# akb825/Cuttlefish

Measured on AMD Instinct MI355X. Metric: Mpixels/s encode, BC7 4096x4096 RGBA8, higher is better.
Workload: dtype u8; 1 GPU; BC7 UNORM Texture::Quality::Normal, one 4096x4096 RGBA8 synthetic photo tile per GPU, resident in HBM; format=BC7, quality=2, blocks_per_launch=1048576, parallelism=surface-per-gpu x1

## Files before the change

cuttlefish_amd/csrc/bc7_encode.hip:

```cpp
#include "cf_device.h"
#include "bc7_packed.h"
#include "bc7_rcp.h"
#include "bc7_roles.h"
#include "bc7_cand.h"

namespace {

#define CF_FRESH_LANE(x) asm volatile("v_mbcnt_lo_u32_b32 %0, -1, 0\n\tv_mbcnt_hi_u32_b32 %0, -1, %0" : "=v"(x))

__device__ __forceinline__ int cf_bperm(int v, uint32_t src)
{
	return __builtin_amdgcn_ds_bpermute((int)(src << 2), v);
}

__device__ const cf_bc7_role_table k_bc7_roles = cf_bc7_make_roles();

__device__ const cf_bc7_cand_table k_bc7_cands = cf_bc7_make_cands();
__device__ const cf_bc7_mask_table k_bc7_masks = cf_bc7_make_masks();

__device__ const cf_bc7_weight_table k_bc7_weights = cf_bc7_make_weights();

__device__ const uint16_t k_part2[64] = CF_BC7_PART2_INIT;

__device__ const uint8_t k_anchor2[64] = {
// ... 216 lines not shown
}

__device__ __forceinline__ uint32_t dot2_u16(uint32_t a, uint32_t b, uint32_t acc)
{
	return __builtin_amdgcn_udot2(__builtin_bit_cast(cf_us2, a), __builtin_bit_cast(cf_us2, b), acc, false);
}

__device__ __forceinline__ void ycc_pairs(uint32_t r, uint32_t g, uint32_t b, uint32_t a, uint32_t& prg, uint32_t& pba)
{
	const uint32_t y = (109u*r + 366u*g + 37u*b + 256u) >> 9;
	prg = y | ((r + 255u - y) << 16);
	pba = (b + 255u - y) | (a << 16);
}

__device__ __forceinline__ uint32_t ycc_pp_sum(const Tex& tx, uint32_t mask, const uint32_t (&yw)[2])
{
	uint32_t pp = 0;
#pragma unroll 1
	for (uint32_t r = 0; r < 4u; ++r) {
		const uint4 ya = *reinterpret_cast<const uint4*>(tx.yc() + 8u*r);
		const uint4 yb = *reinterpret_cast<const uint4*>(tx.yc() + 8u*r + 4u);
		const uint32_t pr[8] = {ya.x, ya.y, ya.z, ya.w, yb.x, yb.y, yb.z, yb.w};
#pragma unroll
		for (int j = 0; j < 4; ++j) {
			const uint32_t t = dot2_u16(pk_mul_u16(pr[2*j], yw[0]), pr[2*j], dot2_u16(pk_mul_u16(pr[2*j + 1], yw[1]), pr[2*j + 1], 0u));
			pp += ((mask >> (4u*r + (uint32_t)j)) & 1u) ? t : 0u;
		}
	}
	return pp;
}

#ifndef CF_BC7_ABLATE
#define CF_BC7_ABLATE 0
#endif
#ifndef CF_BC7_CANDW
#define CF_BC7_CANDW 1
#endif
#ifndef CF_BC7_FITTRIMS
#define CF_BC7_FITTRIMS 3
#endif

#ifndef CF_BC7_DIAG
#define CF_BC7_DIAG 0
#endif
#if CF_BC7_DIAG
enum { CF_DIAG_STARTS, CF_DIAG_STARTS_CACHED, CF_DIAG_STARTS_NARROW, CF_DIAG_PERTURB, CF_DIAG_PERTURB_NARROW,
	CF_DIAG_STARTS_NOPB, CF_DIAG_PERTURB_NOPB, CF_DIAG_PERTURB_PPHIT, CF_DIAG_N };
__device__ unsigned long long cf_bc7_diag[CF_DIAG_N];
#define CF_DIAG_COUNT(i, cond) do { uint32_t l_; CF_FRESH_LANE(l_); if (l_ == 0u && (cond)) atomicAdd(&cf_bc7_diag[i], 1ull); } while (0)
#else
#define CF_DIAG_COUNT(i, cond) do { } while (0)
#endif

struct LaneFit {
	uint32_t q0, q1, pb, err;
	uint32_t w[4];
};

template <bool UNITW, int NK = 8>
__device__ __forceinline__ void assign_lsq_lane(const Tex& tx, uint32_t mask, bool m6,
	uint32_t khalf, uint32_t ib, const uint32_t (&yw)[2], uint32_t pp_sum, bool want_lsq, uint32_t fe0, uint32_t fe1,
	LaneFit& f, float (&nx0)[4], float (&nx1)[4], float (&hq)[3], bool& ok, uint32_t s01 = 0u, uint32_t s23 = 0u)
{
	constexpr bool MINKEY = (CF_BC7_KEYTRIMS & 1) != 0;
	const uint32_t nk = m6 ? 8u : (1u << ib), kbase = m6 ? 8u*khalf : 0u;
	const uint32_t e00 = ub(fe0, 0), e01 = ub(fe0, 1), e02 = ub(fe0, 2), e03 = ub(fe0, 3);
	const uint32_t e10 = ub(fe1, 0), e11 = ub(fe1, 1), e12 = ub(fe1, 2), e13 = ub(fe1, 3);
	uint32_t pal[8], palh[8];
	int base[8];
	uint32_t w03 = 0, w47 = 0;
	if (CF_BC7_FITTRIMS & 2) {
		const uint32_t* wr = k_bc7_weights.w[weight_row(m6, khalf, ib)];
		w03 = wr[0];
		w47 = NK == 8 ? wr[1] : 0u;
	}
	const PalLine line = pal_line(fe0, fe1);
#pragma unroll
	for (int k = 0; k < NK; ++k) {
		const bool valid = ((CF_BC7_FITTRIMS & 2) && k < 4) || (uint32_t)k < nk;
		const uint32_t w = (CF_BC7_FITTRIMS & 2) ? weight_at(w03, w47, (uint32_t)k)
			: bc7_weight(ib, valid ? kbase + (uint32_t)k : 0u);
		const uint32_t iw = 64u - w;
		if (UNITW) {
			pal[k] = (CF_BC7_FITTRIMS & 1) ? pal_at(line, w) : pal_word(fe0, fe1, w);
			palh[k] = 0;
			const int B = (int)((__builtin_amdgcn_udot4(pal[k], pal[k], 0u, false) << 7) | w);
			base[k] = MINKEY ? (valid ? B : CF_BC7_NO_ENTRY) : (valid ? -B : -CF_BC7_NO_ENTRY);
		} else {
			const uint32_t c0 = (__umul24(iw, e00) + __umul24(w, e10) + 32u) >> 6;
			const uint32_t c1 = (__umul24(iw, e01) + __umul24(w, e11) + 32u) >> 6;
			const uint32_t c2 = (__umul24(iw, e02) + __umul24(w, e12) + 32u) >> 6;
			const uint32_t c3 = (__umul24(iw, e03) + __umul24(w, e13) + 32u) >> 6;
			uint32_t qrg, qba;
			ycc_pairs(c0, c1, c2, c3, qrg, qba);
			pal[k] = pk_mul_u16(qrg, yw[0]);
			palh[k] = pk_mul_u16(qba, yw[1]);
			const uint32_t qq = dot2_u16(pal[k], qrg, dot2_u16(palh[k], qba, 0u));
			const int B = (int)((qq << 7) | w);
			base[k] = MINKEY ? (valid ? B : CF_BC7_NO_ENTRY) : (valid ? -B : -CF_BC7_NO_ENTRY);
		}
		asm volatile("" : "+v"(base[k]));
	}
	int m256 = -256;
	if (MINKEY) asm volatile("" : "+s"(m256));
	uint32_t err = pp_sum;
	uint32_t wp0 = 0, wp1 = 0, wp2 = 0, wp3 = 0;
#pragma unroll 1
	for (uint32_t r2 = 0; r2 < 4u; r2 += 2u) {
		uint32_t wpair[2];
#pragma unroll
		for (uint32_t h = 0; h < 2u; ++h) {
			const uint32_t r = r2 + h;
			uint32_t raw[4], rawh[4];
			if (UNITW) {
				const uint4 rw = *reinterpret_cast<const uint4*>(tx.tp() + 4u*r);
				raw[0] = rw.x; raw[1] = rw.y; raw[2] = rw.z; raw[3] = rw.w;
				rawh[0] = rawh[1] = rawh[2] = rawh[3] = 0u;
			} else {
				const uint4 ya = *reinterpret_cast<const uint4*>(tx.yc() + 8u*r);
				const uint4 yb = *reinterpret_cast<const uint4*>(tx.yc() + 8u*r + 4u);
				raw[0] = ya.x; raw[1] = ya.z; raw[2] = yb.x; raw[3] = yb.z;
				rawh[0] = ya.y; rawh[1] = ya.w; rawh[2] = yb.y; rawh[3] = yb.w;
			}
			const uint32_t mrow = (mask >> (4u*r)) & 15u;
			uint32_t wrow = 0;
#pragma unroll
			for (int j = 0; j < 4; ++j) {
				uint32_t rawj = raw[j];
				asm volatile("" : "+v"(rawj), "+v"(wrow));
				const uint32_t p = UNITW ? texel<true>(tx, rawj) : 0u;
				uint32_t key;
				{
					int bestk = MINKEY ? 0x7FFFFFFF : -0x7FFFFFFF;
					const uint32_t prg = rawj, pba = rawh[j];
#pragma unroll
					for (int k = 0; k < NK; ++k) {
						int dt;
						if (UNITW)
							dt = (int)__builtin_amdgcn_udot4(p, pal[k], 0u, false);
						else
							dt = (int)dot2_u16(pba, palh[k], dot2_u16(prg, pal[k], 0u));
						if (MINKEY) {
							const int v = key_min_form(dt, m256, base[k]);
							bestk = v < bestk ? v : bestk;
						} else {
							const int v = key_max_form(dt, base[k]);
							bestk = v > bestk ? v : bestk;
						}
					}
					if (NK == 8) {
						const int other = (int)cf_xor1((uint32_t)bestk);
						bestk = (m6 && (MINKEY ? other < bestk : other > bestk)) ? other : bestk;
					}
					key = (uint32_t)(MINKEY ? bestk : -bestk);
				}
				key = ((mrow >> j) & 1u) ? key : 0u;
				err += (uint32_t)((int)key >> 7);
				wrow |= (key & 127u) << (8*j);
			}
			wpair[h] = wrow;
		}
		wp0 = wp2; wp1 = wp3; wp2 = wpair[0]; wp3 = wpair[1];
	}
	f.err = err;
	f.w[0] = wp0; f.w[1] = wp1; f.w[2] = wp2; f.w[3] = wp3;
	uint32_t S = 0, A = 0, B = 0, C = 0, U[4] = {0, 0, 0, 0}, V[4] = {0, 0, 0, 0};
	if (want_lsq) {
#pragma unroll 1
		for (uint32_t r = 0; r < 4u; ++r) {
			const uint32_t wrow = wp0;
			wp0 = wp1; wp1 = wp2; wp2 = wp3; wp3 = wrow;
			uint32_t P[4];
			uint32_t bo = tx.boff;
			asm volatile("" : "+v"(bo));
			planes<true>(tx, *reinterpret_cast<const uint4*>(tx.plan_ + bo + 4u*r), P);
			S = __builtin_amdgcn_udot4(wrow, 0x01010101u, S, false);
			C = __builtin_amdgcn_udot4(wrow, wrow, C, false);
#pragma unroll
			for (int c = 0; c < 4; ++c)
				V[c] = __builtin_amdgcn_udot4(wrow, P[c], V[c], false);
		}
		A = 4096u*(uint32_t)__builtin_popcount(mask) - 128u*S + C;
		B = 64u*S - C;
		U[0] = 64u*(s01 & 0xFFFFu) - V[0]; U[1] = 64u*(s01 >> 16) - V[1];
		U[2] = 64u*(s23 & 0xFFFFu) - V[2]; U[3] = 64u*(s23 >> 16) - V[3];
	}
	const int det = (int)__umul24((uint32_t)__builtin_popcount(mask), C) - (int)__umul24(S, S);
	ok = det > 0;
	const float inv = rcp_ranged(64.0f*(float)(det > 0 ? det : 1));
	const float fA = (float)A, fB = (float)B, fC = (float)C;
#pragma unroll
	for (int c = 0; c < 4; ++c) {
		if ((tx.chmask >> c) & 1u) {
			const float fU = (float)U[c], fV = (float)V[c];
			const float t0 = fB*fV;
			const float n0 = fmaf(fC, fU, -t0);
			const float t1 = fB*fU;
			const float n1 = fmaf(fA, fV, -t1);
			nx0[c] = n0*inv;
			nx1[c] = n1*inv;
		} else {
			nx0[c] = 0.0f;
			nx1[c] = 0.0f;
		}
	}
	hq[0] = fA; hq[1] = fB; hq[2] = fC;
}

__device__ __forceinline__ void refit_window(const float (&xu0)[4], const float (&xu1)[4], const float (&hq)[3],
	uint32_t cb, uint32_t ab, uint32_t pbk, SubFit& f)
{
	const uint32_t S = pbk ? 1u : 0u;
	const uint32_t P0 = f.pb & 1u, P1 = (f.pb >> 1) & 1u;
// ... 20 lines not shown
			dl1[d] = fb(dw1[d], c) - xu1[c];
		}
		dl0[0] = (lo0 & bm) ? dl0[0] : 1.0e18f;
		dl0[2] = (hi0 & bm) ? dl0[2] : 1.0e18f;
		dl1[0] = (lo1 & bm) ? dl1[0] : 1.0e18f;
		dl1[2] = (hi1 & bm) ? dl1[2] : 1.0e18f;
		float best = 3.0e38f;
		uint32_t bi = 0x11u << (8*c);
#pragma unroll
		for (int i = 0; i < 3; ++i) {
			const float d0 = dl0[i];
			float a0 = fA*d0;
			a0 = a0*d0;
			const float cr = fB2*d0;
#pragma unroll
			for (int j = 0; j < 3; ++j) {
				const float d1 = dl1[j];
				float v = fC*d1;
				v = fmaf(v, d1, a0);
				v = fmaf(cr, d1, v);
				const bool take = v < best;
				best = take ? v : best;
				bi = take ? (uint32_t)(i | (j << 4)) << (8*c) : bi;
			}
		}
		pick |= bi;
	}
	const uint32_t nq0 = f.q0 + (pick & 0x03030303u) - 0x01010101u;
	const uint32_t nq1 = f.q1 + ((pick >> 4) & 0x03030303u) - 0x01010101u;
	const uint32_t ne0 = dequant_word(code_word(nq0, S, P0), tc, ta);
	const uint32_t ne1 = dequant_word(code_word(nq1, S, P1), tc, ta);
	f.q0 = nq0; f.q1 = nq1; f.e0 = ne0; f.e1 = ne1;
}

#define CF_BC7_GEO_WORDS 13
#define CF_BC7_GEO_NONE 0xFFFFFFFFu
__device__ __forceinline__ uint32_t geo_tag(uint32_t id, uint32_t fi) { return id*4u + (id == 0u ? 0u : fi); }

__device__ __forceinline__ uint32_t geo_src(uint32_t id, uint32_t fi, uint32_t wl, bool lay32)
{
	uint32_t s = wl + fi;
	if (id == 0u) s = wl;
	else if (id < 13u) s = fi ? wl + (lay32 ? (id < 5u ? 4u : 1u) : 12u) : wl;
	else if (lay32 && id >= 192u && id < 320u && fi == 2u)
		s = (wl & 32u) + (((wl & 31u) - 11u) >> 1);
	return s & 63u;
}

struct FitStats {
	uint32_t W[CF_MOM_WORDS];
	uint32_t lohi;
};

template <bool UNITW, uint32_t ITERS, int NK = 8, bool GIVEN = false>
__device__ __forceinline__ void fit_lane(const Tex& tx, uint32_t mask, bool m6, uint32_t khalf,
	uint32_t cb, uint32_t ab, uint32_t pbk, uint32_t ib, const uint32_t (&wt)[4],
	const uint32_t (&yw)[2], bool scalar, float frac, uint32_t* gbase, uint32_t gmode, uint32_t gsrc, const FitStats& gs, LaneFit& best)
{
	float axis[4], mean[4];
	float tmin, tmax;
	uint32_t lo, hi, pp_sum, s01, s23;
	if (gmode == 2u) {
		const uint32_t* gc = gbase + gsrc;
#pragma unroll
		for (int c = 0; c < 4; ++c) {
			axis[c] = __uint_as_float(gc[c*CF_WG_THREADS]);
			mean[c] = __uint_as_float(gc[(4 + c)*CF_WG_THREADS]);
		}
		tmin = __uint_as_float(gc[8*CF_WG_THREADS]);
		tmax = __uint_as_float(gc[9*CF_WG_THREADS]);
		const uint32_t lh = gc[10*CF_WG_THREADS];
		lo = lh & 255u; hi = lh >> 8;
		pp_sum = gc[11*CF_WG_THREADS];
		const float fn = (float)__builtin_popcount(mask);
		s01 = (uint32_t)(mean[0]*fn + 0.5f) | ((uint32_t)(mean[1]*fn + 0.5f) << 16);
		s23 = (uint32_t)(mean[2]*fn + 0.5f) | ((uint32_t)(mean[3]*fn + 0.5f) << 16);
	} else {
		const uint32_t n = (uint32_t)__builtin_popcount(mask);
		uint32_t s[4] = {0, 0, 0, 0};
		uint32_t q00 = 0, q01 = 0, q02 = 0, q03 = 0, q11 = 0, q12 = 0, q13 = 0, q22 = 0, q23 = 0,
			q33 = 0;
		lo = 255u; hi = 0u;
		if (GIVEN && gmode == 3u) {
			uint32_t q[10];
			mom_unpack(gs.W, s, q);
			q00 = q[0]; q01 = q[1]; q02 = q[2]; q03 = q[3]; q11 = q[4]; q12 = q[5]; q13 = q[6]; q22 = q[7]; q23 = q[8]; q33 = q[9];
			lo = gs.lohi & 255u; hi = gs.lohi >> 8;
		} else
#pragma unroll 1
		for (uint32_t r = 0; r < 4u; ++r) {
			uint32_t P[4];
			const uint4 pr = *reinterpret_cast<const uint4*>(tx.pl() + 4u*r);
			planes<true>(tx, pr, P);
			const uint32_t a4 = tx.rot == 0u ? pr.w : (tx.rot == 1u ? pr.x : (tx.rot == 2u ? pr.y : pr.z));
#pragma unroll
			for (int j = 0; j < 4; ++j) {
				const uint32_t a = (a4 >> (8*j)) & 255u;
				lo = a < lo ? a : lo;
				hi = a > hi ? a : hi;
			}
			const uint32_t m4 = bytemask4((mask >> (4u*r)) & 15u);
			const uint32_t M0 = P[0] & m4, M1 = P[1] & m4, M2 = P[2] & m4, M3 = P[3] & m4;
			s[0] = __builtin_amdgcn_udot4(M0, 0x01010101u, s[0], false);
			s[1] = __builtin_amdgcn_udot4(M1, 0x01010101u, s[1], false);
			s[2] = __builtin_amdgcn_udot4(M2, 0x01010101u, s[2], false);
			s[3] = __builtin_amdgcn_udot4(M3, 0x01010101u, s[3], false);
			q00 = __builtin_amdgcn_udot4(M0, P[0], q00, false);
			q01 = __builtin_amdgcn_udot4(M0, P[1], q01, false);
			q02 = __builtin_amdgcn_udot4(M0, P[2], q02, false);
			q03 = __builtin_amdgcn_udot4(M0, P[3], q03, false);
// ... 12 lines not shown

		float bestd = C00;
		float v0 = C00, v1 = C01, v2 = C02, v3 = C03;
		if (C11 > bestd) { bestd = C11; v0 = C01; v1 = C11; v2 = C12; v3 = C13; }
		if (C22 > bestd) { bestd = C22; v0 = C02; v1 = C12; v2 = C22; v3 = C23; }
		if (C33 > bestd) { bestd = C33; v0 = C03; v1 = C13; v2 = C23; v3 = C33; }
#pragma unroll
		for (int it = 0; it < 3; ++it) {
			float r0 = C00*v0; r0 = fmaf(C01, v1, r0); r0 = fmaf(C02, v2, r0); r0 = fmaf(C03, v3, r0);
			float r1 = C01*v0; r1 = fmaf(C11, v1, r1); r1 = fmaf(C12, v2, r1); r1 = fmaf(C13, v3, r1);
			float r2 = C02*v0; r2 = fmaf(C12, v1, r2); r2 = fmaf(C22, v2, r2); r2 = fmaf(C23, v3, r2);
			float r3 = C03*v0; r3 = fmaf(C13, v1, r3); r3 = fmaf(C23, v2, r3); r3 = fmaf(C33, v3, r3);
			v0 = r0; v1 = r1; v2 = r2; v3 = r3;
		}
		const float mx = fmaxf(fmaxf(fabsf(v0), fabsf(v1)), fmaxf(fabsf(v2), fabsf(v3)));
#pragma unroll
		for (int c = 0; c < 4; ++c) axis[c] = 0.0f;
		if (mx > 0.0f) {
			const float im = rcp_tested(mx);
			v0 = v0*im; v1 = v1*im; v2 = v2*im; v3 = v3*im;
			float l2 = v0*v0;
			l2 = fmaf(v1, v1, l2);
			l2 = fmaf(v2, v2, l2);
			l2 = fmaf(v3, v3, l2);
			const float is = rcp_ranged(sqrtf(l2));
			axis[0] = v0*is; axis[1] = v1*is; axis[2] = v2*is; axis[3] = v3*is;
		}

		const float in = inv_n(n);
#pragma unroll
		for (int c = 0; c < 4; ++c)
			mean[c] = (float)s[c]*in;
		tmin = 3.0e38f; tmax = -3.0e38f;
#pragma unroll 1
		for (uint32_t r = 0; r < 4u; ++r) {
			const uint4 rw = *reinterpret_cast<const uint4*>(tx.tp() + 4u*r);
			const uint32_t raw[4] = {rw.x, rw.y, rw.z, rw.w};
			const uint32_t mrow = (mask >> (4u*r)) & 15u;
#pragma unroll
			for (int j = 0; j < 4; ++j) {
				const uint32_t p = texel<true>(tx, raw[j]);
				const bool m = (mrow >> j) & 1u;
				float t = axis[0]*(fb(p, 0) - mean[0]);
				t = fmaf(axis[1], fb(p, 1) - mean[1], t);
				t = fmaf(axis[2], fb(p, 2) - mean[2], t);
				t = fmaf(axis[3], fb(p, 3) - mean[3], t);
				tmin = m ? fminf(tmin, t) : tmin;
				tmax = m ? fmaxf(tmax, t) : tmax;
			}
		}
		pp_sum = UNITW ? q00 + q11 + q22 + q33 : ycc_pp_sum(tx, mask, yw);
		s01 = s[0] | (s[1] << 16);
		s23 = s[2] | (s[3] << 16);
		if (GIVEN ? gmode != 0u : gmode == 1u) {
			uint32_t lane;
			CF_FRESH_LANE(lane);
			uint32_t* gc = gbase + lane;
#pragma unroll
			for (int c = 0; c < 4; ++c) {
				gc[c*CF_WG_THREADS] = __float_as_uint(axis[c]);
				gc[(4 + c)*CF_WG_THREADS] = __float_as_uint(mean[c]);
			}
			gc[8*CF_WG_THREADS] = __float_as_uint(tmin);
			gc[9*CF_WG_THREADS] = __float_as_uint(tmax);
			gc[10*CF_WG_THREADS] = lo | (hi << 8);
			gc[11*CF_WG_THREADS] = pp_sum;
		}
	}
	{
		const float d = (tmax - tmin)*frac;
		tmin = tmin + d;
		tmax = tmax - d;
	}
	float x0[4], x1[4];
#pragma unroll
	for (int c = 0; c < 4; ++c) {
		x0[c] = clamp255(fmaf(axis[c], tmin, mean[c]));
		x1[c] = clamp255(fmaf(axis[c], tmax, mean[c]));
	}
	if (scalar) {
		const float flo = (float)lo, fhi = (float)hi;
		const float d = (fhi - flo)*frac;
		x0[0] = 0.0f; x0[1] = 0.0f; x0[2] = 0.0f; x0[3] = clamp255(flo + d);
		x1[0] = 0.0f; x1[1] = 0.0f; x1[2] = 0.0f; x1[3] = clamp255(fhi - d);
	}
	uint32_t geo = cb | (ab << 4) | (pbk << 8) | (ib << 12);
	asm volatile("" : "+v"(geo));
#define G_CB (geo & 15u)
#define G_AB ((geo >> 4) & 15u)
#define G_PBK ((geo >> 8) & 15u)
#define G_IB (geo >> 12)
	SubFit q;
	quantize<UNITW>(x0, x1, G_CB, G_AB, G_PBK, wt, q);
	best.q0 = q.q0; best.q1 = q.q1; best.pb = q.pb;
	bool live;
	float hq[3];
	assign_lsq_lane<UNITW, NK>(tx, mask, m6, khalf, G_IB, yw, pp_sum, ITERS > 0u, q.e0, q.e1, best, x0, x1, hq, live, s01, s23);
#pragma unroll 1
	for (uint32_t r = 0; r < ITERS; ++r) {
		LaneFit cur;
		bool ok;
		asm volatile("" : "+v"(geo));
		{
			float c0[4], c1[4];
#pragma unroll
			for (int c = 0; c < 4; ++c) {
				c0[c] = clamp255(x0[c]);
				c1[c] = clamp255(x1[c]);
			}
			quantize<UNITW>(c0, c1, G_CB, G_AB, G_PBK, wt, q);
		}
		if (!(CF_BC7_ABLATE & 8)) refit_window(x0, x1, hq, G_CB, G_AB, G_PBK, q);
		cur.q0 = q.q0; cur.q1 = q.q1; cur.pb = q.pb;
		assign_lsq_lane<UNITW, NK>(tx, mask, m6, khalf, G_IB, yw, pp_sum, r + 1u < ITERS, q.e0, q.e1, cur, x0, x1, hq, ok, s01, s23);
		const bool better = live && cur.err < best.err;
		if (better)
			best = cur;
		live = better && ok;
	}
#undef G_CB
#undef G_AB
#undef G_PBK
#undef G_IB
}

__device__ __forceinline__ uint32_t w2i(uint32_t w, uint32_t ib)
{
	return (w*((1u << ib) - 1u) + 32u) >> 6;
}

__device__ __forceinline__ uint4 pack_block_group(const uint32_t* wcol, uint32_t id, uint32_t lane,
	bool pair)
{
	const uint32_t h = lane >> 5, hl = pair ? (lane & 31u) : lane, hbase = pair ? (lane & 32u) : 0u;
	if (CF_BC7_ABLATE & 64) {
		uint4 r;
		r.x = id; r.y = wcol[0]; r.z = wcol[CF_WG_THREADS]; r.w = h;
		return r;
	}
	uint32_t mode, part = 0, rot = 0, isel = 0;
	if (id == 0u) mode = 6;
	else if (id < 5u) { mode = 5; rot = id - 1u; }
	else if (id < 13u) { mode = 4; rot = (id - 5u) & 3u; isel = (id - 5u) >> 2; }
	else if (id < 128u) { mode = 1; part = id - 64u; }
	else if (id < 192u) { mode = 3; part = id - 128u; }
	else if (id < 256u) { mode = 0; part = id - 192u; }
	else if (id < 320u) { mode = 2; part = id - 256u; }
	else { mode = 7; part = id - 320u; }
	const uint32_t ns  = (0x21112323u >> (4u*mode)) & 15u;
	const uint32_t pbn = (0x60006664u >> (4u*mode)) & 15u;
	const uint32_t cb  = (0x57757564u >> (4u*mode)) & 15u;
	const uint32_t ab  = (0x57860000u >> (4u*mode)) & 15u;
	const uint32_t pk  = (0x11001021u >> (4u*mode)) & 15u;
	const uint32_t ib  = (0x24222233u >> (4u*mode)) & 15u;
	const uint32_t ib2 = (0x00230000u >> (4u*mode)) & 15u;
	uint32_t ibc = ib, iba = ib2;
	const bool swapsets = mode == 4u && isel != 0u;
	if (swapsets) { ibc = 3u; iba = 2u; }
	const uint32_t p2 = k_part2[part], p3 = k_part3[part];
	uint32_t a1 = 0, a2 = 0;
	if (ns == 2u) a1 = k_anchor2[part];
	else if (ns == 3u) { a1 = k_anchor3a[part]; a2 = k_anchor3b[part]; }

	const uint32_t t = hl & 15u;
	const uint32_t sb = ns == 1u ? 0u : (ns == 2u ? ((p2 >> t) & 1u) : ((p3 >> (2u*t)) & 3u));
	const uint32_t wv = (wcol[(7u + (t >> 2))*CF_WG_THREADS] >> (8u*(t & 3u))) & 255u;
	const uint32_t ws = (wcol[(11u + (t >> 2))*CF_WG_THREADS] >> (8u*(t & 3u))) & 255u;
// ... 576 lines not shown
					case 0: cb = 4; ab = 0; pbk = 1; ib = 3; break;
					case 2: cb = 5; ab = 0; pbk = 0; ib = 2; break;
					default: cb = 5; ab = 5; pbk = 1; ib = 2; break;
				}
				const uint32_t sp2 = k_part2[mypart], sp3 = k_part3[mypart];
				if (st == 0u)
					mask = sub ? sp2 : (~sp2 & 0xFFFFu);
				else
					mask = part3_mask(sp3, sub);
				active = true;
			}
			if (CF_BC7_ABLATE & 1) active = active && (m6 || plane);
			if (CF_BC7_ABLATE & 2) active = active && !plane;
#if CF_BC7_DIAG
			const bool nopb = __ballot(active && pbk != 0u) == 0ull;
			CF_DIAG_COUNT(CF_DIAG_STARTS_NOPB, sst && nopb);
#endif
			uint32_t wl[4] = {wt[0], wt[1], wt[2], wt[3]};
			if (!UNITW && rot) {
				const uint32_t t3 = wl[3];
				if (rot == 1u) { wl[3] = wl[0]; wl[0] = t3; }
				else if (rot == 2u) { wl[3] = wl[1]; wl[1] = t3; }
				else { wl[3] = wl[2]; wl[2] = t3; }
			}
			const uint32_t chm = (sst || words) ? chm_s : (m6 ? 15u : (sca ? 8u : (vecp ? 7u : (H_ALPHA ? 15u : 7u))));
			const uint32_t wv[4] = {(chm & 1u) ? wl[0] : 0u, (chm & 2u) ? wl[1] : 0u,
				(chm & 4u) ? wl[2] : 0u, (chm & 8u) ? wl[3] : 0u};
			LaneFit lf;
			lf.err = 0; lf.q0 = 0; lf.q1 = 0; lf.pb = 0;
#pragma unroll
			for (int k = 0; k < 4; ++k) lf.w[k] = 0;
			const uint32_t yw[2] = {(chm & 7u) ? ywrg : 0u,
				((chm & 7u) ? (ywba & 0xFFFFu) : 0u) | ((chm & 8u) ? (ywba & 0xFFFF0000u) : 0u)};
			FitStats gs;
			if (given && st == 0u) {
				const uint32_t blk = B_OFF >> 4;
				uint32_t T[CF_MOM_WORDS];
#pragma unroll
				for (int m = 0; m < CF_MOM_WORDS; ++m) T[m] = mom[__umul24(blk, CF_BC7_MOM_WORDS) + (uint32_t)m];
				gs.lohi = lohi[blk*4u + ((rot + 3u) & 3u)];
				if (quality >= 1u && plane) {
					const uint32_t* sc = ((pair && mypart >= 32u) ? gbase : cbase) + (pair ? L_HBASE + (mypart & 31u) : mypart);
#pragma unroll
					for (int m = 0; m < CF_MOM_WORDS; ++m) gs.W[m] = sc[m*CF_WG_THREADS];
					if (sub == 0u) {
						mom_sub(T, gs.W, gs.W);
						asm volatile("" : "+v"(gs.W[0]));
					}
				} else
					mom_whole(T, !(H_ALPHA), rot, chm, gs.W);
				__builtin_amdgcn_wave_barrier();
				gmode = 3u;
			}
			if (active) {
				if (narrow)
					fit_lane<UNITW, iters, 4>(make_tex(tile, plan, yccp, B_OFF, rot, chm), mask, m6, lane & 1u, cb, ab, pbk, ib,
						wv, yw, sca, frac, gbase, gmode, gsrc, gs, lf);
				else
					fit_lane<UNITW, iters, 8, given>(make_tex(tile, plan, yccp, B_OFF, rot, chm), mask, m6, lane & 1u, cb, ab, pbk, ib,
						wv, yw, sca, frac, gbase, gmode, gsrc, gs, lf);
			}
			CF_FRESH_LANE(lane);
			if (sst) {
				const uint32_t k2 = koff + (lay32 ? (L_HL >> 3) : (lane >> 4));
				const uint32_t wl2 = TOP_LANE(k2 & 7u);
				const uint32_t id2 = cbase[wl2 + 19*CF_WG_THREADS], cerr2 = cbase[wl2 + 18*CF_WG_THREADS];
				const bool n32 = lay32 && (CF_BC7_CANDW ? CF_CAND_NS(cbase[wl2 + 6*CF_WG_THREADS]) == 3u : id2 >= 192u && id2 < 320u);
				const uint32_t j82 = L_HL & 7u;
				const uint32_t v2 = lay32 ? (n32 ? (j82 >= 3u ? 1u : 0u) : (L_HL >> 1) & 3u) : (lane >> 2) & 3u;
				const uint32_t fi2 = lay32 ? (n32 ? (j82 >= 6u ? 3u : j82 - 3u*v2) : (L_HL & 1u)) : (lane & 3u);
				const uint32_t err02 = cbase[TOP_LANE(0u) + 18*CF_WG_THREADS];
				const FitGeo g2 = column_geo(cbase + wl2, id2, fi2);
				const uint32_t kf2 = g2.m6 ? 0u : fi2;
				const bool active2 = L_SLOT_OK && k2 < ntop && cerr2 != 0xFFFFFFFFu && err02 != 0u && (g2.m6 ? fi2 < 2u : fi2 < g2.nfits);
				uint32_t skey = active2 ? ((lf.err << 2) | v2) : 0xFFFFFFFFu;
				{
					const uint32_t o1 = (uint32_t)cf_bperm((int)skey, n32 ? (j82 < 3u ? lane + 3u : (j82 < 6u ? lane - 3u : lane)) : lane ^ (lay32 ? 2u : 4u));
					skey = o1 < skey ? o1 : skey;
					const uint32_t o2 = (uint32_t)cf_bperm((int)skey, n32 ? lane : lane ^ (lay32 ? 4u : 8u));
					skey = o2 < skey ? o2 : skey;
				}
				uint32_t* wc = cbase + wl2;
				const uint32_t cur_err = wc[(15u + kf2)*CF_WG_THREADS];
				const bool win = active2 && skey == ((lf.err << 2) | v2) && lf.err < cur_err && (!g2.m6 || fi2 == 0u);
#pragma unroll 1
				for (uint32_t j = 0; j < 3u; ++j) {
					if (win && kf2 == j)
						column_put_fit(wc, g2, kf2, lf.q0, lf.q1, lf.pb, lf.w, lf.err);
					__builtin_amdgcn_wave_barrier();
				}
				continue;
			}
			uint32_t best_err;
			if constexpr (words) {
				const uint32_t rw = R_WORDS[0];
				bool act = CF_ROLE_ACTIVE(rw, UNITW) != 0u;
				if (CF_BC7_ABLATE & 1) act = act && (rw & (CF_ROLE_M6 | CF_ROLE_PLANE)) != 0u;
				if (CF_BC7_ABLATE & 2) act = act && (rw & CF_ROLE_PLANE) == 0u;
				const uint32_t cidv = CF_ROLE_IDB(rw) + mypart;
				if (act || st == 0u)
					gbase[lane + 12*CF_WG_THREADS] = act ? cidv*4u + CF_ROLE_KF(rw) : CF_BC7_GEO_NONE;
				const uint32_t s1 = (lane + 1u) & 63u;
				const uint32_t s2 = (lay32 ? (lane & 32u) : 0u) + CF_ROLE_S2(rw);
				const uint32_t m1 = 0u - CF_ROLE_USE1(rw), mv = 0u - ((rw / CF_ROLE_VECP) & 1u), m2 = 0u - CF_ROLE_USE2(rw);
				const uint32_t m3 = m2 & ~mv, m4 = (mv & 0xFF000000u) | m3;
				const uint32_t e1 = (uint32_t)cf_bperm((int)lf.err, s1), e2 = (uint32_t)cf_bperm((int)lf.err, s2);
				const uint32_t a01 = (uint32_t)cf_bperm((int)lf.q0, s1), a11 = (uint32_t)cf_bperm((int)lf.q1, s1);
				const uint32_t a02 = (uint32_t)cf_bperm((int)lf.q0, s2), a12 = (uint32_t)cf_bperm((int)lf.q1, s2);
				const uint32_t pb1 = (uint32_t)cf_bperm((int)lf.pb, s1), pb2 = (uint32_t)cf_bperm((int)lf.pb, s2);
				uint32_t w1[4], w2[4];
#pragma unroll
				for (int k = 0; k < 4; ++k) {
					w1[k] = (uint32_t)cf_bperm((int)lf.w[k], s1);
// ... 160 lines not shown
			const bool nopb = __ballot(act && g.pbk != 0u) == 0ull;
			CF_DIAG_COUNT(CF_DIAG_PERTURB_NOPB, !(CF_BC7_ABLATE & 32) && (kk == ntop ? uber2 : uber) != 0u && nopb);
#endif
			CF_DIAG_COUNT(CF_DIAG_PERTURB_PPHIT, !(CF_BC7_ABLATE & 32) && (kk == ntop ? uber2 : uber) != 0u && pphit);
			const uint32_t S = g.pbk ? 1u : 0u;
			const uint32_t fq0 = g.planes45 ? (g.sca ? 4u : 0u) : 2u*kf, fq1 = fq0 + 1u;
#pragma unroll 1
			for (uint32_t r = 0; r < ((CF_BC7_ABLATE & 32) ? 0u : (kk == ntop ? uber2 : uber)); ++r) {
				bool moved = false;
#pragma unroll 1
				for (uint32_t set = 0; set < 2u; ++set) {
					if (!((msets >> set) & 1u))
						continue;
					const uint32_t q0 = wc[fq0*CF_WG_THREADS], q1 = wc[fq1*CF_WG_THREADS];
					const uint32_t pbv = g.planes45 ? 0u : (wc[6*CF_WG_THREADS] >> (2u*kf)) & 3u;
					const uint32_t cur_err = wc[(15u + kf)*CF_WG_THREADS];
					bool valid = act;
					uint32_t nq0 = q0, nq1 = q1, npb = pbv;
					if (set == 0u) {
						const uint32_t e = mv >> 3, ch = (mv >> 1) & 3u, up = mv & 1u;
						const uint32_t bits_c = ch < 3u ? g.cb : g.ab;
						if (bits_c) {
							const uint32_t src = e ? q1 : q0;
							const int nv = (int)((src >> (8u*ch)) & 255u) + (up ? 1 : -1);
							valid = valid && nv >= 0 && nv <= (int)((1u << bits_c) - 1u);
							const uint32_t nw = (src & ~(255u << (8u*ch))) | (((uint32_t)nv & 255u) << (8u*ch));
							nq0 = e ? q0 : nw;
							nq1 = e ? nw : q1;
						} else if (g.pbk == 1u && e == 0u)
							npb = pbv ^ (1u << up);
						else if (g.pbk == 2u && e == 0u && up == 0u)
							npb = pbv ^ 3u;
						else
							valid = false;
					} else {
						const uint32_t ch = mv >> 2, k4 = mv & 3u;
						const uint32_t bits_c = ch < 3u ? g.cb : g.ab;
						const int d0 = (k4 == 0u || k4 == 2u) ? 1 : -1, d1 = (k4 == 0u || k4 == 3u) ? 1 : -1;
						const int v0 = (int)((q0 >> (8u*ch)) & 255u) + d0, v1 = (int)((q1 >> (8u*ch)) & 255u) + d1;
						const int qm = (int)((1u << bits_c) - 1u);
						valid = valid && bits_c != 0u && v0 >= 0 && v0 <= qm && v1 >= 0 && v1 <= qm;
						nq0 = (q0 & ~(255u << (8u*ch))) | (((uint32_t)v0 & 255u) << (8u*ch));
						nq1 = (q1 & ~(255u << (8u*ch))) | (((uint32_t)v1 & 255u) << (8u*ch));
					}
					LaneFit f;
					f.q0 = nq0; f.q1 = nq1; f.pb = npb; f.err = 0;
					const uint32_t tc = g.cb ? g.cb + S : 0u, ta = g.ab ? g.ab + S : 0u;
					const uint32_t fe0 = dequant_word(code_word(nq0, S, npb & S), tc, ta);
					const uint32_t fe1 = dequant_word(code_word(nq1, S, (npb >> 1) & S), tc, ta);
#pragma unroll
					for (int j = 0; j < 4; ++j) f.w[j] = 0;
					float x0[4], x1[4], hq[3];
					bool okk;
					if (narrow)
						assign_lsq_lane<UNITW, 4>(tx, g.mask, g.m6, L_HL & 1u, g.ib, yw, pp_sum, false, fe0, fe1, f, x0, x1, hq, okk);
					else
						assign_lsq_lane<UNITW>(tx, g.mask, g.m6, L_HL & 1u, g.ib, yw, pp_sum, false, fe0, fe1, f, x0, x1, hq, okk);
					const uint32_t key = valid ? ((f.err << 4) | mv) : 0xFFFFFFFFu;
					uint32_t fitmin = cf_row_min_u32(key);
					if (g.m6) {
						const uint32_t other = (uint32_t)cf_bperm((int)fitmin, lane ^ 16u);
						fitmin = other < fitmin ? other : fitmin;
					}
					const bool win = valid && key == fitmin && f.err < cur_err && (!g.m6 || (L_HL & 1u) == 0u);
#pragma unroll 1
					for (uint32_t j = 0; j < 3u; ++j) {
						if (win && kf == j)
							column_put_fit(wc, g, kf, nq0, nq1, npb, f.w, f.err);
						__builtin_amdgcn_wave_barrier();
					}
					moved = moved || __ballot(win) != 0ull;
				}
				if (!moved)
					break;
			}
			CF_FRESH_LANE(lane);
			if (lane == wl && L_CSLOT[18*CF_WG_THREADS] != 0xFFFFFFFFu)
				L_CSLOT[18*CF_WG_THREADS] = L_CSLOT[15*CF_WG_THREADS] + L_CSLOT[16*CF_WG_THREADS] + L_CSLOT[17*CF_WG_THREADS];
			__builtin_amdgcn_wave_barrier();
		}
	}
	CF_FRESH_LANE(lane);
	const uint32_t win_id = cbase[win_lane + 19*CF_WG_THREADS];
	return pack_block_group(cbase + win_lane, win_id, lane, pair);
#undef H_ALPHA
#undef H_GATE
#undef ANY_OPAQUE
#undef TOP_LANE
#undef B_TP
#undef B_OFF
#undef L_H
#undef L_HBASE
#undef L_HL
#undef L_SLOT_OK
#undef L_CSLOT
}

}

#ifndef CF_BC7_WAVES
#define CF_BC7_WAVES(UNITW, WIDE) ((UNITW) ? 4 : 3)
#endif
template <int PIX, bool UNITW, bool WIDE, int LEVEL>
__global__ void __launch_bounds__(CF_WG_THREADS)
__attribute__((amdgpu_waves_per_eu(CF_BC7_WAVES(UNITW, WIDE), CF_BC7_WAVES(UNITW, WIDE))))
cfhip_bc7_encode_kernel(cf_kparams kp)
{
	__shared__ uint32_t cands[CF_BC7_CAND_WORDS*CF_WG_THREADS];
	__shared__ uint32_t geoc[CF_BC7_GEO_WORDS*CF_WG_THREADS];
	__shared__ __attribute__((aligned(16))) uint32_t tile[CF_BLOCKS_PER_WG*16];
// ... 107 lines not shown
```

cuttlefish_amd/csrc/bc7_packed.h:

```cpp
#ifndef CFHIP_BC7_PACKED_H
#define CFHIP_BC7_PACKED_H

#include <stdint.h>

#if defined(__HIPCC__)
#define CF_PK __host__ __device__ __forceinline__
#else
#define CF_PK static inline
#endif
#if defined(__HIP_DEVICE_COMPILE__)
#define CF_PK_MUL24(a, b) __umul24((a), (b))
#else
#define CF_PK_MUL24(a, b) ((a)*(b))
#endif

#ifndef CF_BC7_KEYTRIMS
#define CF_BC7_KEYTRIMS 3
#endif

#if defined(__HIP_DEVICE_COMPILE__)
#define CF_PK_MUL24S(a, b) __mul24((a), (b))
#else
#define CF_PK_MUL24S(a, b) ((a)*(b))
#endif

#define CF_BC7_NO_ENTRY 0x3FFFFFFF
CF_PK int key_max_form(int dt, int negB) { return (dt << 8) + negB; }
CF_PK int key_min_form(int dt, int m256, int B) { return CF_PK_MUL24S(dt, m256) + B; }

CF_PK uint32_t dequant1(uint32_t v, uint32_t t)
{
	return CF_PK_MUL24(v, (1u << t) + 1u) >> (2u*t - 8u);
}

CF_PK uint32_t dequant_rgb(uint32_t word, uint32_t t)
{
	const uint32_t c3 = word & 0x00FFFFFFu;
	const uint32_t low = ((1u << (8u - t)) - 1u)*0x010101u;
	return (c3 << (8u - t)) | ((c3 >> (2u*t - 8u)) & low);
}

CF_PK uint32_t dequant_word(uint32_t word, uint32_t tc, uint32_t ta)
{
	const uint32_t coded = (tc ? 0x00FFFFFFu : 0u) | (ta ? 0xFF000000u : 0u);
	return (dequant_rgb(word, tc ? tc : 8u) | (dequant1(word >> 24, ta ? ta : 8u) << 24)) & coded;
}

CF_PK uint32_t code_word(uint32_t qword, uint32_t S, uint32_t P)
{
	return (qword << S) | (P ? 0x01010101u : 0u);
}

CF_PK uint32_t pal_word(uint32_t e0, uint32_t e1, uint32_t w)
{
	const uint32_t iw = 64u - w;
	const uint32_t m = 0x00FF00FFu, half = 0x00200020u;
	const uint32_t rb = CF_PK_MUL24(iw, e0 & m) + CF_PK_MUL24(w, e1 & m) + half;
	const uint32_t ga = CF_PK_MUL24(iw, (e0 >> 8) & m) + CF_PK_MUL24(w, (e1 >> 8) & m) + half;
	return ((rb >> 6) & m) | ((ga << 2) & ~m);
}

struct PalLine { uint32_t rb0, rbd, ga0, gad; };

CF_PK PalLine pal_line(uint32_t e0, uint32_t e1)
{
	const uint32_t m = 0x00FF00FFu, half = 0x00200020u;
	const uint32_t a_rb = e0 & m, a_ga = (e0 >> 8) & m;
	PalLine l;
	l.rb0 = (a_rb << 6) + half; l.rbd = (e1 & m) - a_rb;
	l.ga0 = (a_ga << 6) + half; l.gad = ((e1 >> 8) & m) - a_ga;
	return l;
}

CF_PK uint32_t pal_at(const PalLine& l, uint32_t w)
{
	const uint32_t m = 0x00FF00FFu;
	const uint32_t rb = l.rb0 + w*l.rbd;
	const uint32_t ga = l.ga0 + w*l.gad;
	return ((rb >> 6) & m) | ((ga << 2) & ~m);
}

// ... 73 lines not shown
```

Baseline: 2924 Mpixels/s.

## Compute BC7 palette index dot products with MFMA i8 4x4x4 instead of udot4

Replaces the per-texel udot4 loop over palette entries with a matrix-core v_mfma_i32_4x4x4i8 per palette entry, computing dot products for four texels of a row at once. Inputs are recentred to signed bytes via xor 0x80 with a compensating base term, and palette channels are permuted for rotation. Weights are stored as full bytes and packed with v_perm. Because MFMA needs the whole wavefront, inactive lanes now enter the fit path and have their results zeroed, and global cache writes are restricted to owner lanes. This trades scalar VALU dot work for matrix-core throughput, at the cost of extra wave divergence work and operand loads.

```diff
diff --git a/cuttlefish_amd/csrc/bc7_encode.hip b/cuttlefish_amd/csrc/bc7_encode.hip
--- a/cuttlefish_amd/csrc/bc7_encode.hip
+++ b/cuttlefish_amd/csrc/bc7_encode.hip
@@ -292,17 +292,34 @@
 #define CF_DIAG_COUNT(i, cond) do { } while (0)
 #endif
 
+typedef int cf_int4 __attribute__((ext_vector_type(4)));
+template <bool UNITW>
+__device__ __forceinline__ void arow_load(const uint32_t* tile, uint32_t boff, uint32_t (&arow)[4])
+{
+	arow[0] = arow[1] = arow[2] = arow[3] = 0u;
+	if (UNITW && (CF_BC7_KEYTRIMS & 1) && (CF_BC7_MFMADOT & 1)) {
+		uint32_t lane;
+		CF_FRESH_LANE(lane);
+#pragma unroll
+		for (uint32_t r = 0; r < 4u; ++r)
+			arow[r] = tile[boff + 4u*r + (lane & 3u)] ^ 0x80808080u;
+	}
+}
+
 struct LaneFit {
 	uint32_t q0, q1, pb, err;
 	uint32_t w[4];
 };
 
-template <bool UNITW, int NK = 8>
+template <bool UNITW, int NK = 8, int CBSZ = 3>
 __device__ __forceinline__ void assign_lsq_lane(const Tex& tx, uint32_t mask, bool m6,
-	uint32_t khalf, uint32_t ib, const uint32_t (&yw)[2], uint32_t pp_sum, bool want_lsq, uint32_t fe0, uint32_t fe1,
+	uint32_t khalf, uint32_t ib, const uint32_t (&yw)[2], uint32_t pp_sum, bool want_lsq, uint32_t fe0, uint32_t fe1, const uint32_t (&arow)[4],
 	LaneFit& f, float (&nx0)[4], float (&nx1)[4], float (&hq)[3], bool& ok, uint32_t s01 = 0u, uint32_t s23 = 0u)
 {
 	constexpr bool MINKEY = (CF_BC7_KEYTRIMS & 1) != 0;
+	constexpr bool WBYTE = UNITW && MINKEY && (CF_BC7_MFMADOT & 4) != 0;
+	constexpr int WBITS = WBYTE ? 8 : 7;
+	constexpr bool MFMA = UNITW && MINKEY && (CF_BC7_MFMADOT & 1) != 0;
 	const uint32_t nk = m6 ? 8u : (1u << ib), kbase = m6 ? 8u*khalf : 0u;
 	const uint32_t e00 = ub(fe0, 0), e01 = ub(fe0, 1), e02 = ub(fe0, 2), e03 = ub(fe0, 3);
 	const uint32_t e10 = ub(fe1, 0), e11 = ub(fe1, 1), e12 = ub(fe1, 2), e13 = ub(fe1, 3);
@@ -314,7 +331,8 @@
 		w03 = wr[0];
 		w47 = NK == 8 ? wr[1] : 0u;
 	}
-	const PalLine line = pal_line(fe0, fe1);
+	const uint32_t rsel = tx.rot == 0u ? 0x03020100u : (tx.rot == 1u ? 0x00020103u : (tx.rot == 2u ? 0x01020300u : 0x02030100u));
+	const PalLine line = MFMA ? pal_line(__builtin_amdgcn_perm(fe0, fe0, rsel), __builtin_amdgcn_perm(fe1, fe1, rsel)) : pal_line(fe0, fe1);
 #pragma unroll
 	for (int k = 0; k < NK; ++k) {
 		const bool valid = ((CF_BC7_FITTRIMS & 2) && k < 4) || (uint32_t)k < nk;
@@ -324,7 +342,11 @@
 		if (UNITW) {
 			pal[k] = (CF_BC7_FITTRIMS & 1) ? pal_at(line, w) : pal_word(fe0, fe1, w);
 			palh[k] = 0;
-			const int B = (int)((__builtin_amdgcn_udot4(pal[k], pal[k], 0u, false) << 7) | w);
+			int B = (int)((__builtin_amdgcn_udot4(pal[k], pal[k], 0u, false) << WBITS) | w);
+			if (MFMA) {
+				B = mfma_entry_base(B, __builtin_amdgcn_udot4(pal[k], 0x01010101u, 0u, false), WBITS + 1);
+				pal[k] ^= 0x80808080u;
+			}
 			base[k] = MINKEY ? (valid ? B : CF_BC7_NO_ENTRY) : (valid ? -B : -CF_BC7_NO_ENTRY);
 		} else {
 			const uint32_t c0 = (__umul24(iw, e00) + __umul24(w, e10) + 32u) >> 6;
@@ -341,8 +363,8 @@
 		}
 		asm volatile("" : "+v"(base[k]));
 	}
-	int m256 = -256;
-	if (MINKEY) asm volatile("" : "+s"(m256));
+	int kfac = WBYTE ? -512 : -256;
+	if (MINKEY) asm volatile("" : "+s"(kfac));
 	uint32_t err = pp_sum;
 	uint32_t wp0 = 0, wp1 = 0, wp2 = 0, wp3 = 0;
 #pragma unroll 1
@@ -363,25 +385,44 @@
 				rawh[0] = ya.y; rawh[1] = ya.w; rawh[2] = yb.y; rawh[3] = yb.w;
 			}
 			const uint32_t mrow = (mask >> (4u*r)) & 15u;
-			uint32_t wrow = 0;
+			uint32_t wrow = 0, krow[4];
+			int bestm[4] = {0x7FFFFFFF, 0x7FFFFFFF, 0x7FFFFFFF, 0x7FFFFFFF};
+			if (MFMA) {
+				cf_int4 cop;
+				cop.x = (int)__builtin_amdgcn_udot4(raw[0], 0x80808080u, 0u, false);
+				cop.y = (int)__builtin_amdgcn_udot4(raw[1], 0x80808080u, 0u, false);
+				cop.z = (int)__builtin_amdgcn_udot4(raw[2], 0x80808080u, 0u, false);
+				cop.w = (int)__builtin_amdgcn_udot4(raw[3], 0x80808080u, 0u, false);
+				const uint32_t aop = r2 == 0u ? (h == 0u ? arow[0] : arow[1]) : (h == 0u ? arow[2] : arow[3]);
+#pragma unroll
+				for (int k = 0; k < NK; ++k) {
+					const cf_int4 d = __builtin_amdgcn_mfma_i32_4x4x4i8((int)aop, (int)pal[k], cop, CBSZ, 0, 0);
+					const int v0 = key_min_form(d.x, kfac, base[k]), v1 = key_min_form(d.y, kfac, base[k]);
+					const int v2 = key_min_form(d.z, kfac, base[k]), v3 = key_min_form(d.w, kfac, base[k]);
+					bestm[0] = v0 < bestm[0] ? v0 : bestm[0]; bestm[1] = v1 < bestm[1] ? v1 : bestm[1];
+					bestm[2] = v2 < bestm[2] ? v2 : bestm[2]; bestm[3] = v3 < bestm[3] ? v3 : bestm[3];
+				}
+			}
 #pragma unroll
 			for (int j = 0; j < 4; ++j) {
 				uint32_t rawj = raw[j];
-				asm volatile("" : "+v"(rawj), "+v"(wrow));
-				const uint32_t p = UNITW ? texel<true>(tx, rawj) : 0u;
+				if (MFMA) { }
+				else if (WBYTE) asm volatile("" : "+v"(rawj));
+				else asm volatile("" : "+v"(rawj), "+v"(wrow));
+				const uint32_t p = (UNITW && !MFMA) ? texel<true>(tx, rawj) : 0u;
 				uint32_t key;
 				{
-					int bestk = MINKEY ? 0x7FFFFFFF : -0x7FFFFFFF;
+					int bestk = MFMA ? bestm[j] : (MINKEY ? 0x7FFFFFFF : -0x7FFFFFFF);
 					const uint32_t prg = rawj, pba = rawh[j];
 #pragma unroll
-					for (int k = 0; k < NK; ++k) {
+					for (int k = 0; k < (MFMA ? 0 : NK); ++k) {
 						int dt;
 						if (UNITW)
 							dt = (int)__builtin_amdgcn_udot4(p, pal[k], 0u, false);
 						else
 							dt = (int)dot2_u16(pba, palh[k], dot2_u16(prg, pal[k], 0u));
 						if (MINKEY) {
-							const int v = key_min_form(dt, m256, base[k]);
+							const int v = key_min_form(dt, kfac, base[k]);
 							bestk = v < bestk ? v : bestk;
 						} else {
 							const int v = key_max_form(dt, base[k]);
@@ -395,10 +436,11 @@
 					key = (uint32_t)(MINKEY ? bestk : -bestk);
 				}
 				key = ((mrow >> j) & 1u) ? key : 0u;
-				err += (uint32_t)((int)key >> 7);
-				wrow |= (key & 127u) << (8*j);
-			}
-			wpair[h] = wrow;
+				err += (uint32_t)((int)key >> WBITS);
+				if (WBYTE) krow[j] = key;
+				else wrow |= (key & 127u) << (8*j);
+			}
+			wpair[h] = WBYTE ? key_row_weights(krow[0], krow[1], krow[2], krow[3]) : wrow;
 		}
 		wp0 = wp2; wp1 = wp3; wp2 = wpair[0]; wp3 = wpair[1];
 	}
@@ -525,10 +567,10 @@
 	uint32_t lohi;
 };
 
-template <bool UNITW, uint32_t ITERS, int NK = 8, bool GIVEN = false>
+template <bool UNITW, uint32_t ITERS, int NK = 8, bool GIVEN = false, int CBSZ = 3>
 __device__ __forceinline__ void fit_lane(const Tex& tx, uint32_t mask, bool m6, uint32_t khalf,
 	uint32_t cb, uint32_t ab, uint32_t pbk, uint32_t ib, const uint32_t (&wt)[4],
-	const uint32_t (&yw)[2], bool scalar, float frac, uint32_t* gbase, uint32_t gmode, uint32_t gsrc, const FitStats& gs, LaneFit& best)
+	const uint32_t (&yw)[2], bool scalar, float frac, uint32_t* gbase, uint32_t gmode, uint32_t gsrc, const FitStats& gs, bool owner, LaneFit& best)
 {
 	float axis[4], mean[4];
 	float tmin, tmax;
@@ -647,7 +689,7 @@
 		pp_sum = UNITW ? q00 + q11 + q22 + q33 : ycc_pp_sum(tx, mask, yw);
 		s01 = s[0] | (s[1] << 16);
 		s23 = s[2] | (s[3] << 16);
-		if (GIVEN ? gmode != 0u : gmode == 1u) {
+		if ((GIVEN ? gmode != 0u : gmode == 1u) && ((UNITW && (CF_BC7_KEYTRIMS & 1) && (CF_BC7_MFMADOT & 1)) ? owner : true)) {
 			uint32_t lane;
 			CF_FRESH_LANE(lane);
 			uint32_t* gc = gbase + lane;
@@ -690,7 +732,9 @@
 	best.q0 = q.q0; best.q1 = q.q1; best.pb = q.pb;
 	bool live;
 	float hq[3];
-	assign_lsq_lane<UNITW, NK>(tx, mask, m6, khalf, G_IB, yw, pp_sum, ITERS > 0u, q.e0, q.e1, best, x0, x1, hq, live, s01, s23);
+	uint32_t arow[4];
+	arow_load<UNITW>(tx.tile_, tx.boff, arow);
+	assign_lsq_lane<UNITW, NK, CBSZ>(tx, mask, m6, khalf, G_IB, yw, pp_sum, ITERS > 0u, q.e0, q.e1, arow, best, x0, x1, hq, live, s01, s23);
 #pragma unroll 1
 	for (uint32_t r = 0; r < ITERS; ++r) {
 		LaneFit cur;
@@ -707,7 +751,8 @@
 		}
 		if (!(CF_BC7_ABLATE & 8)) refit_window(x0, x1, hq, G_CB, G_AB, G_PBK, q);
 		cur.q0 = q.q0; cur.q1 = q.q1; cur.pb = q.pb;
-		assign_lsq_lane<UNITW, NK>(tx, mask, m6, khalf, G_IB, yw, pp_sum, r + 1u < ITERS, q.e0, q.e1, cur, x0, x1, hq, ok, s01, s23);
+		arow_load<UNITW>(tx.tile_, tx.boff, arow);
+		assign_lsq_lane<UNITW, NK, CBSZ>(tx, mask, m6, khalf, G_IB, yw, pp_sum, r + 1u < ITERS, q.e0, q.e1, arow, cur, x0, x1, hq, ok, s01, s23);
 		const bool better = live && cur.err < best.err;
 		if (better)
 			best = cur;
@@ -1390,13 +1435,19 @@
 				__builtin_amdgcn_wave_barrier();
 				gmode = 3u;
 			}
-			if (active) {
+			constexpr bool wholewave = UNITW && (CF_BC7_KEYTRIMS & 1) && (CF_BC7_MFMADOT & 1);
+			if (wholewave ? __ballot(active) != 0ull : active) {
 				if (narrow)
-					fit_lane<UNITW, iters, 4>(make_tex(tile, plan, yccp, B_OFF, rot, chm), mask, m6, lane & 1u, cb, ab, pbk, ib,
-						wv, yw, sca, frac, gbase, gmode, gsrc, gs, lf);
+					fit_lane<UNITW, iters, 4, false, WIDE ? 4 : 3>(make_tex(tile, plan, yccp, B_OFF, rot, chm), mask, m6, lane & 1u, cb, ab, pbk, ib,
+						wv, yw, sca, frac, gbase, gmode, gsrc, gs, active, lf);
 				else
-					fit_lane<UNITW, iters, 8, given>(make_tex(tile, plan, yccp, B_OFF, rot, chm), mask, m6, lane & 1u, cb, ab, pbk, ib,
-						wv, yw, sca, frac, gbase, gmode, gsrc, gs, lf);
+					fit_lane<UNITW, iters, 8, given, WIDE ? 4 : 3>(make_tex(tile, plan, yccp, B_OFF, rot, chm), mask, m6, lane & 1u, cb, ab, pbk, ib,
+						wv, yw, sca, frac, gbase, gmode, gsrc, gs, active, lf);
+				if (wholewave && !active) {
+					lf.err = 0; lf.q0 = 0; lf.q1 = 0; lf.pb = 0;
+#pragma unroll
+					for (int k = 0; k < 4; ++k) lf.w[k] = 0;
+				}
 			}
 			CF_FRESH_LANE(lane);
 			if (sst) {
@@ -1663,10 +1714,12 @@
 					for (int j = 0; j < 4; ++j) f.w[j] = 0;
 					float x0[4], x1[4], hq[3];
 					bool okk;
+					uint32_t arow[4];
+					arow_load<UNITW>(tx.tile_, tx.boff, arow);
 					if (narrow)
-						assign_lsq_lane<UNITW, 4>(tx, g.mask, g.m6, L_HL & 1u, g.ib, yw, pp_sum, false, fe0, fe1, f, x0, x1, hq, okk);
+						assign_lsq_lane<UNITW, 4, WIDE ? 4 : 3>(tx, g.mask, g.m6, L_HL & 1u, g.ib, yw, pp_sum, false, fe0, fe1, arow, f, x0, x1, hq, okk);
 					else
-						assign_lsq_lane<UNITW>(tx, g.mask, g.m6, L_HL & 1u, g.ib, yw, pp_sum, false, fe0, fe1, f, x0, x1, hq, okk);
+						assign_lsq_lane<UNITW, 8, WIDE ? 4 : 3>(tx, g.mask, g.m6, L_HL & 1u, g.ib, yw, pp_sum, false, fe0, fe1, arow, f, x0, x1, hq, okk);
 					const uint32_t key = valid ? ((f.err << 4) | mv) : 0xFFFFFFFFu;
 					uint32_t fitmin = cf_row_min_u32(key);
 					if (g.m6) {
diff --git a/cuttlefish_amd/csrc/bc7_packed.h b/cuttlefish_amd/csrc/bc7_packed.h
--- a/cuttlefish_amd/csrc/bc7_packed.h
+++ b/cuttlefish_amd/csrc/bc7_packed.h
@@ -27,6 +27,24 @@
 #define CF_BC7_NO_ENTRY 0x3FFFFFFF
 CF_PK int key_max_form(int dt, int negB) { return (dt << 8) + negB; }
 CF_PK int key_min_form(int dt, int m256, int B) { return CF_PK_MUL24S(dt, m256) + B; }
+
+#ifndef CF_BC7_MFMADOT
+#define CF_BC7_MFMADOT 5
+#endif
+
+CF_PK int mfma_entry_base(int B, uint32_t sb, int fbits)
+{
+	return B + (int)(512u << (7 + fbits)) - (int)CF_PK_MUL24(sb, 1u << (7 + fbits));
+}
+
+CF_PK uint32_t key_row_weights(uint32_t k0, uint32_t k1, uint32_t k2, uint32_t k3)
+{
+#if defined(__HIP_DEVICE_COMPILE__)
+	return __builtin_amdgcn_perm(k1, k0, 0x0C0C0400u) | __builtin_amdgcn_perm(k3, k2, 0x04000C0Cu);
+#else
+	return (k0 & 255u) | ((k1 & 255u) << 8) | ((k2 & 255u) << 16) | ((k3 & 255u) << 24);
+#endif
+}
 
 CF_PK uint32_t dequant1(uint32_t v, uint32_t t)
 {
```

Measured after the change: 3016 Mpixels/s (median of 6 runs). +3.1%, better.
